# pierluigiferrari/ssd_keras

Hardware: AMD Instinct MI355X
Metric: images/sec SSD300 fwd+decode @batch32 (higher is better)
Workload: dtype f32 (decode, threshold, TF-style f32 NMS, top-k); bf16 conv backbone; 1 GPU; SSD300 VGG-16 inference (mode='inference': forward + DecodeDetections), 21 classes, batch 32 per GPU, conf 0.01 / NMS 0.45 / top-200, random-init weights, synthetic 300x300x3 uint8-range images; per_gpu_batch=32, global_batch=32, conv_dtype=bf16, parallelism=replicas x1, launch=hip_graph (forward + DecodeDetections captured once, replayed per step), decode_stream=same stream; DecodeDetections reads the head outputs directly (no y_pred in HBM)

## Files before the change

include/ssdhip.h:

```cpp
#ifndef SSDHIP_H
#define SSDHIP_H

#include <stddef.h>

#ifdef __cplusplus
extern "C" {
#endif

#define SSDHIP_ABI_VERSION 1

enum {
    SSDHIP_OK = 0,
    SSDHIP_E_BADARG = -1,
    SSDHIP_E_WORKSPACE = -2,
    SSDHIP_E_LAUNCH = -3
};

enum { SSDHIP_F32 = 0, SSDHIP_F64 = 1 };
enum { SSDHIP_CENTROIDS = 0, SSDHIP_CORNERS = 1, SSDHIP_MINMAX = 2 };
enum { SSDHIP_BORDER_HALF = 0, SSDHIP_BORDER_INCLUDE = 1, SSDHIP_BORDER_EXCLUDE = 2 };
enum {
    SSDHIP_SEM_NUMPY = 0,
    SSDHIP_SEM_KERAS = 1,
    SSDHIP_SEM_DEBUG = 2
};

int ssdhip_abi_version(void);
const char* ssdhip_strerror(int rc);

size_t ssdhip_decode_workspace_bytes(int B, int N, int C, int top_k, int nms_cap, int class_agnostic, int in_dtype);
int ssdhip_decode_detections(const void* y_pred, int in_dtype, int B, int N, int C,
                             double conf_thresh, double iou_thresh, int top_k, int nms_cap,
                             int class_agnostic, int semantics,
                             int coords, int normalize_coords, double img_height, double img_width,
                             int border_pixels,
                             void* out, int out_dtype, int out_rows, int* out_count, int* out_anchor_idx,
                             void* ws, size_t ws_bytes, void* stream);
int ssdhip_decode_stages(int stages, const void* y_pred, int in_dtype, int B, int N, int C,
                         double conf_thresh, double iou_thresh, int top_k, int nms_cap,
                         int class_agnostic, int semantics,
                         int coords, int normalize_coords, double img_height, double img_width,
                         int border_pixels,
                         void* out, int out_dtype, int out_rows, int* out_count, int* out_anchor_idx,
                         void* ws, size_t ws_bytes, void* stream);

size_t ssdhip_encode_workspace_bytes(int B, int N, int C, int G_total);
int ssdhip_encode(const double* anchors, const double* variances, const double* gt, const int* gt_offsets,
                  int G_total, int max_gt_per_image, int B, int N, int C, double img_height, double img_width,
                  int matching_type, double pos_iou_threshold, double neg_iou_limit,
                  int coords, int normalize_coords, int border_pixels, int background_id,
                  float* y_encoded_f32, double* y_encoded_f64, int* match_gt,
                  void* ws, size_t ws_bytes, void* stream);

// ... 488 lines not shown
```

ssd_keras_amd/_native.py:

```python
from __future__ import annotations

import ctypes
import os
import threading

import numpy as np

_LIB_PATH = os.environ.get("SSDHIP_LIB") or os.path.join(os.path.dirname(os.path.abspath(__file__)), "libssdhip.so")
_lib = None
_lock = threading.Lock()

F32, F64 = 0, 1
COORDS = {"centroids": 0, "corners": 1, "minmax": 2}
BORDER = {"half": 0, "include": 1, "exclude": 2}
SEM_NUMPY, SEM_KERAS, SEM_DEBUG = 0, 1, 2
ABI_VERSION = 1


class SsdHipError(RuntimeError):
    pass


def lib_path():
    return _LIB_PATH
# ... 33 lines not shown
                ("photo_prob", ctypes.c_double * 4), ("photo_lower", ctypes.c_double * 4), ("photo_upper", ctypes.c_double * 4),
                ("patch_prob", ctypes.c_double),
                ("min_scale", ctypes.c_double), ("max_scale", ctypes.c_double),
                ("min_aspect_ratio", ctypes.c_double), ("max_aspect_ratio", ctypes.c_double),
                ("n_trials", ctypes.c_int), ("clip_boxes", ctypes.c_int), ("criterion", ctypes.c_int), ("n_boxes_min", ctypes.c_int),
                ("validator_lower", ctypes.c_double), ("validator_upper", ctypes.c_double),
                ("filter_lower", ctypes.c_double), ("filter_upper", ctypes.c_double),
                ("flip_prob", ctypes.c_double),
                ("out_height", ctypes.c_int), ("out_width", ctypes.c_int), ("interpolation", ctypes.c_int),
                ("resize_min_area", ctypes.c_double)]


class _SatAugParams(ctypes.Structure):
    _fields_ = [("var", _VarAugParams), ("vflip_prob", ctypes.c_double), ("rotate_prob", ctypes.c_double)]


_I, _LL, _SZ, _D, _F, _P = ctypes.c_int, ctypes.c_longlong, ctypes.c_size_t, ctypes.c_double, ctypes.c_float, ctypes.c_void_p
_INTP, _PARAMS, _PHOTO = ctypes.POINTER(ctypes.c_int), ctypes.POINTER(_AugParams), ctypes.POINTER(_AugPhoto)
_LLP = ctypes.POINTER(ctypes.c_longlong)
SIGNATURES = {
    "ssdhip_abi_version": (_I, []),
    "ssdhip_strerror": (ctypes.c_char_p, [_I]),
    "ssdhip_decode_workspace_bytes": (_SZ, [_I] * 7),
    "ssdhip_decode_detections": (_I, [_P] + [_I] * 4 + [_D, _D] + [_I] * 6 + [_D, _D, _I, _P, _I, _I] + [_P] * 3 + [_SZ, _P]),
    "ssdhip_decode_stages": (_I, [_I, _P] + [_I] * 4 + [_D, _D] + [_I] * 6 + [_D, _D, _I, _P, _I, _I] + [_P] * 3 + [_SZ, _P]),
    "ssdhip_encode_workspace_bytes": (_SZ, [_I] * 4),
    "ssdhip_encode": (_I, [_P] * 4 + [_I] * 5 + [_D, _D, _I, _D, _D] + [_I] * 4 + [_P] * 4 + [_SZ, _P]),
    "ssdhip_loss_workspace_bytes": (_SZ, [_I] * 3),
    "ssdhip_loss_forward": (_I, [_P, _P] + [_I] * 5 + [_F] + [_P] * 4 + [_SZ, _P]),
    "ssdhip_loss_backward": (_I, [_P] * 5 + [_I] * 3 + [_F, _P, _P]),
    "ssdhip_convert_coordinates": (_I, [_P, _I, _P, _LL] + [_I] * 4 + [_P]),
    "ssdhip_iou_result_dtype": (_I, [_I] * 3),
    "ssdhip_box_overlap": (_I, [_I, _P, _I, _I, _P] + [_I] * 5 + [_P, _P]),
    "ssdhip_match_bipartite_greedy": (_I, [_P, _I, _I, _P, _P]),
    "ssdhip_match_multi_workspace_bytes": (_SZ, [_I, _I]),
    "ssdhip_match_multi": (_I, [_P, _I, _I, _D] + [_P] * 4 + [_SZ, _P]),
    "ssdhip_greedy_nms_workspace_bytes": (_SZ, [_I]),
    "ssdhip_greedy_nms": (_I, [_P] + [_I] * 4 + [_P, _I, _D, _I, _I] + [_P] * 3 + [_SZ, _P]),
    "ssdhip_box_filter": (_I, [_P] * 3 + [_I] * 6 + [_D] * 3 + [_I, _P, _P]),
    "ssdhip_match_predictions_workspace_bytes": (_SZ, [_I, _I]),
    "ssdhip_match_predictions": (_I, [_P, _P, _I] + [_P] * 3 + [_I, _I, _D, _I] + [_P] * 6 + [_SZ, _P]),
    "ssdhip_match_predictions_multi": (_I, [_P] * 3 + [_I] + [_P] * 3 + [_I, _I, _P, _I, _D, _I] + [_P] * 6 + [_SZ, _P]),
    "ssdhip_coco_match_workspace_bytes": (_SZ, [_I] * 4),
    "ssdhip_coco_match": (_I, [_P] * 3 + [_I] + [_P] * 4 + [_I, _I, _P, _I, _P, _I, _I] + [_P] * 8 + [_SZ, _P]),
    "ssdhip_coco_accumulate_workspace_bytes": (_SZ, [_I, _I]),
    "ssdhip_coco_accumulate": (_I, [_P] * 4 + [_I, _P, _P] + [_I] * 4 + [_P, _I, _I, _P, _I] + [_P] * 4 + [_SZ, _P]),
# ... 192 lines not shown
    check(rc, name)
    return True


def launch(name, device, *args):
    _launch(name, device, args)


def _launch_or_none(name, device, *args):
    return _launch(name, device, args, declines=True)


class _Workspaces:

    def __init__(self):
        self._bufs = {}

    def get(self, device, purpose, nbytes, zeroed=False):
        torch = _torch()
        key = (str(device), purpose, int(torch.cuda.current_stream(device).cuda_stream))
        buf = self._bufs.get(key)
        if buf is None or buf.numel() < nbytes:
            buf = (torch.zeros if zeroed else torch.empty)(int(nbytes), dtype=torch.uint8, device=device)
            self._bufs[key] = buf
        return buf


workspaces = _Workspaces()


def decode(y_pred, conf_thresh, iou_thresh, top_k, nms_cap, class_agnostic, semantics, coords, normalize_coords,
           img_height, img_width, border_pixels, out_dtype, out_rows, want_anchor_idx=False, workspace=None,
           stages=7, outputs=None):
    torch = _torch()
    lib = load()
    require_cuda(y_pred, "y_pred")
    if y_pred.dtype not in (torch.float32, torch.float64):
        raise SsdHipError("y_pred must be float32 or float64")
    in_dt = F32 if y_pred.dtype == torch.float32 else F64
    if in_dt == F64 and semantics == SEM_KERAS:
        raise SsdHipError("the DecodeDetections layers are float32 graphs: float64 predictions are not accepted there")
    B, N, L = y_pred.shape
    C = L - 12
    dev = y_pred.device
    k = int(top_k) if top_k else 0
    cap = int(nms_cap) if nms_cap else 0
    need = lib.ssdhip_decode_workspace_bytes(B, N, C, k, cap, int(bool(class_agnostic)), in_dt)
    if need == 0:
        raise SsdHipError("unsupported decode shape B=%d N=%d C=%d" % (B, N, C))
    ws = workspace if workspace is not None else workspaces.get(dev, "decode", need)
    if outputs is not None:
        out, count, aidx = outputs
    else:
        out = torch.empty((B, out_rows, 6), dtype=torch.float64 if out_dtype == F64 else torch.float32, device=dev)
        count = torch.empty((B,), dtype=torch.int32, device=dev)
        aidx = torch.empty((B, out_rows), dtype=torch.int32, device=dev) if want_anchor_idx else None
    launch("ssdhip_decode_stages", dev, int(stages), ctypes.c_void_p(y_pred.data_ptr()), in_dt, B, N, C, float(conf_thresh),
           float(iou_thresh), k, cap, int(bool(class_agnostic)), int(semantics), COORDS[coords], int(bool(normalize_coords)),
           float(img_height if img_height is not None else 1.0), float(img_width if img_width is not None else 1.0), BORDER[border_pixels],
           ctypes.c_void_p(out.data_ptr()), out_dtype, int(out_rows), ctypes.c_void_p(count.data_ptr()),
           ctypes.c_void_p(aidx.data_ptr()) if aidx is not None else None, ctypes.c_void_p(ws.data_ptr()), ws.numel())
    return out, count, aidx


def to_device(a, device=None, dtype=None):
    torch = _torch()
    if isinstance(a, np.ndarray):
        a = torch.from_numpy(np.ascontiguousarray(a))
    if device is None:
        device = a.device if a.is_cuda else torch.device("cuda", torch.cuda.current_device())
    if dtype is not None and a.dtype != dtype:
        a = a.to(dtype)
    return a.to(device, non_blocking=False).contiguous()




def _nhwc_bf16(t, name):
    torch = _torch()
    if not t.is_cuda or t.dtype != torch.bfloat16 or t.dim() != 4:
        raise SsdHipError("%s must be a 4-D bfloat16 CUDA tensor" % name)
    if not t.permute(0, 2, 3, 1).is_contiguous():
        t = t.contiguous(memory_format=torch.channels_last)
        if not t.permute(0, 2, 3, 1).is_contiguous():
# ... 223 lines not shown


def assemble_predictions(confs, locs, conf_biases, loc_biases, n_boxes, anchors_var, n_classes):
    torch = _torch()
    args, keep, B, N = _head_sources(confs, locs, conf_biases, loc_biases, n_boxes, anchors_var, n_classes)
    y = torch.empty((B, N, n_classes + 12), dtype=torch.float32, device=confs[0].device)
    f32 = confs[0].dtype == torch.float32
    launch("ssdhip_assemble_predictions_strided_" + ("f32" if f32 else "bf16"), y.device, *args, B, N, int(n_classes), _ptr(y))
    return y


def decode_from_heads(confs, locs, conf_biases, loc_biases, n_boxes, anchors_var, n_classes, conf_thresh, iou_thresh, top_k,
                      nms_cap, class_agnostic, semantics, coords, normalize_coords, img_height, img_width, border_pixels, out_dtype,
                      out_rows, want_anchor_idx=False):
    torch = _torch()
    lib = load()
    args, keep, B, N = _head_sources(confs, locs, conf_biases, loc_biases, n_boxes, anchors_var, n_classes)
    dev = confs[0].device
    k = int(top_k) if top_k else 0
    cap = int(nms_cap) if nms_cap else 0
    need = lib.ssdhip_decode_workspace_bytes(B, N, int(n_classes), k, cap, int(bool(class_agnostic)), F32)
    if need == 0:
        raise SsdHipError("unsupported decode shape B=%d N=%d C=%d" % (B, N, n_classes))
    ws = workspaces.get(dev, "decode", need)
    out = torch.empty((B, out_rows, 6), dtype=torch.float64 if out_dtype == F64 else torch.float32, device=dev)
    count = torch.empty((B,), dtype=torch.int32, device=dev)
    aidx = torch.empty((B, out_rows), dtype=torch.int32, device=dev) if want_anchor_idx else None
    launch("ssdhip_decode_from_heads_f32" if confs[0].dtype == torch.float32 else "ssdhip_decode_from_heads", dev, *args, B, N,
           int(n_classes), float(conf_thresh), float(iou_thresh), k, cap, int(bool(class_agnostic)), int(semantics), COORDS[coords],
           int(bool(normalize_coords)), float(img_height if img_height is not None else 1.0),
           float(img_width if img_width is not None else 1.0), BORDER[border_pixels], _ptr(out), out_dtype, int(out_rows), _ptr(count),
           _ptr(aidx), _ptr(ws), ws.numel())
    return out, count, aidx


def channel_sums_partial(gy):
    torch = _torch()
    lib = load()
    gy, (b, h, w, c) = _nhwc_bf16(gy, "gy")
    nb = lib.ssdhip_relu_bwd_bias_blocks(b * h * w, c)
    if nb == 0:
        return None
    partial = torch.empty((nb, c), dtype=torch.float32, device=gy.device)
    launch("ssdhip_channel_sums_nhwc_bf16", gy.device, _ptr(gy), _ptr(partial), b * h * w, c, nb)
    return partial


def relu_bwd_bias(gy, y, reduce=True):
    torch = _torch()
    lib = load()
    gy, (b, h, w, c) = _nhwc_bf16(gy, "gy")
    y, _ = _nhwc_bf16(y, "y")
    nb = lib.ssdhip_relu_bwd_bias_blocks(b * h * w, c)
    if nb == 0:
        return None
# ... 1994 lines not shown
```

ssd_keras_amd/csrc/ssdhip_decode.hip:

```cpp
#include <hip/hip_runtime.h>
#include <stdint.h>
#include <stdlib.h>

#include "ssdhip.h"
#include "ssdhip_math.h"
#include "ssdhip_tile.h"
#include "ssdhip_heads.h"
#include "ssdhip_decode64.h"

#ifdef SSDHIP_PROFILE
__device__ unsigned long long g_prof[64];
#define PROF_DECL long long _pt = clock64(); long long _pa[12] = {0, 0, 0, 0, 0, 0, 0, 0, 0, 0, 0, 0};
#define PROF_MARK(i) { const long long _t = clock64(); _pa[i] += _t - _pt; _pt = _t; }
#define PROF_FLUSH(base) if (threadIdx.x == 0) { for (int _i = 0; _i < 12; ++_i) if (_pa[_i]) atomicAdd(&g_prof[(base) + _i], (unsigned long long)_pa[_i]); }
extern "C" int ssdhip_profile_read(unsigned long long* host_out, int reset) {
    if (hipMemcpyFromSymbol(host_out, HIP_SYMBOL(g_prof), sizeof(g_prof)) != hipSuccess) return -1;
    if (reset) { unsigned long long z[64] = {0}; if (hipMemcpyToSymbol(HIP_SYMBOL(g_prof), z, sizeof(z)) != hipSuccess) return -1; }
    return 0;
}
#else
#define PROF_DECL
#define PROF_MARK(i)
#define PROF_FLUSH(base)
#endif

// ... 635 lines not shown
__device__ __forceinline__ void load_keys_cached(const u64* keys, int n, int tid, int first, u64 (&kc)[KP]) {
#if defined(__HIP_DEVICE_COMPILE__)
    int nn = n;
    asm volatile("" : "+s"(nn));
    const __amdgpu_buffer_rsrc_t rs = __builtin_amdgcn_make_buffer_rsrc(const_cast<u64*>(keys), 0, nn * 8, 0x00020000);
#pragma unroll
    for (int u = 0; u < KP; ++u) {
        const u32x2 v = __builtin_amdgcn_raw_buffer_load_b64(rs, tid * 8, (first + u) * T * 8, 0);
        const u64 key = ((u64)v.y << 32) | v.x;
        kc[u] = key ? key : ~0ull;
    }
#endif
}

__device__ __forceinline__ int uni32(int v) { return __builtin_amdgcn_readfirstlane(v); }
__device__ __forceinline__ u64 uni64(u64 v) {
    return ((u64)(u32)__builtin_amdgcn_readfirstlane((int)(u32)(v >> 32)) << 32) | (u64)(u32)__builtin_amdgcn_readfirstlane((int)(u32)v);
}

#ifndef SSDHIP_NMS_WAVES512
#define SSDHIP_NMS_WAVES512 6
#endif
template <int POL, int T, bool FULL>
__global__ __launch_bounds__(T, (T >= 512 ? SSDHIP_NMS_WAVES512 : 3)) void nms_kernel(DecodeParams p, const float4* __restrict__ boxes,
                                               const u64* __restrict__ cand, const int* __restrict__ cand_count,
                                               const int* __restrict__ work_order,
                                               u64* __restrict__ kept, int* __restrict__ kept_count, int redo_only) {
    constexpr int W = T / 64;
    constexpr int KC = KC_KEYS / T;
    constexpr int KP = 9;
    static_assert(KC % KP == 0, "KC must be a multiple of the trip size");
    constexpr int UA = T >= 512 ? (POL == POL_NUMPY64 ? 2 : 4) : 4, UB = T >= 512 ? 2 : 4;
    constexpr bool PREFETCH = T < 512;
    const int total_work = p.B * p.G;
    const int per_xcd = (total_work + 7) >> 3;
    int work = (blockIdx.x & 7) * per_xcd + (blockIdx.x >> 3);
    if ((int)(blockIdx.x >> 3) >= per_xcd || work >= total_work) return;
    if (work_order) work = work_order[work];
    if (redo_only && kept_count[work] != -1) return;
    const int b = work / p.G;

    __shared__ __attribute__((aligned(16))) u64 keybuf[MAX_CHUNK + 8];
    __shared__ __attribute__((aligned(16))) u64 keybuf2[MAX_CHUNK + 8];
    __shared__ int fill2;
    constexpr size_t SCRATCH = sizeof(FBox) * MAX_CHUNK > NMS_NBINS * sizeof(u32) ? sizeof(FBox) * MAX_CHUNK : NMS_NBINS * sizeof(u32);
    __shared__ __attribute__((aligned(16))) unsigned char scratch[SCRATCH];
    __shared__ __attribute__((aligned(16))) float4 cf4[POL == POL_NUMPY64 ? MAX_CHUNK : 1];
    __shared__ FBox kb[KEPT_LDS + 8 * W + 8];
    __shared__ __attribute__((aligned(16))) float4 kf4[POL == POL_NUMPY64 ? KEPT_LDS : 1];
    __shared__ u64 maskrow[64];
    __shared__ u64 supp_a[W];
    __shared__ int red[264];
    __shared__ int fill;
    u32* hist = reinterpret_cast<u32*>(scratch);
    FBox* cb = reinterpret_cast<FBox*>(scratch);
    u64* sorted = keybuf;

    const int tid = threadIdx.x, lane = tid & 63, wave = tid >> 6;
    const int n = cand_count[work];
    const u64* keys = cand + (size_t)work * p.N;
    u64* kept_out = kept + (size_t)work * p.cap_store;
    const float4* img_boxes = boxes + (size_t)b * p.N;
// ... 101 lines not shown
                    else if (m2 > 0 && bin >= bin_cut2) keybuf2[atomicAdd(&fill2, 1)] = key;
                }
            }
        } else {
            for (int i0 = tid; i0 < n; i0 += 8 * T) {
                u64 k8[8];
#pragma unroll
                for (int u = 0; u < 8; ++u) { const int i = i0 + u * T; k8[u] = i < n ? keys[i] : ~0ull; }
#pragma unroll
                for (int u = 0; u < 8; ++u) {
                    const u64 key = k8[u];
                    if (!(key < upper)) continue;
                    const int bin = bin_of<NMS_BIN_SHIFT, NMS_NBINS>((u32)(key >> IDX_BITS), p.thr_key);
                    const bool take = by_bin ? (bin >= bin_cut) : (key >= cutoff);
                    if (take) keybuf[atomicAdd(&fill, 1)] = key;
                    else if (m2 > 0 && bin >= bin_cut2) keybuf2[atomicAdd(&fill2, 1)] = key;
                }
            }
        }
        pending2 = m2;
        __syncthreads();
        PROF_MARK(1)
        }
        {
            constexpr int PER = MAX_CHUNK / T;
            u64 v[PER];
#pragma unroll
            for (int r = 0; r < PER; ++r) v[r] = keybuf[tid * PER + r];
            block_bitonic_desc_regs<T, PER>(v, reinterpret_cast<u64*>(scratch));
#pragma unroll
            for (int r = 0; r < PER; ++r) keybuf[tid * PER + r] = v[r];
            __syncthreads();
        }
        PROF_MARK(2)
        upper = uni64(sorted[m - 1]);
        has_upper = true;
        consumed += m;
        for (int i = tid; i < m; i += T) {
            const u32 idx = IDX_MASK - (u32)(sorted[i] & IDX_MASK);
            const float4 f4 = img_boxes[idx];
            cb[i] = make_fbox<POL>(f4, idx, k);
            if (POL == POL_NUMPY64) cf4[i] = f4;
        }
        __syncthreads();
        PROF_MARK(3)

        for (int base = 0; base < m && K < cap_eff && !finished; base += 64) {
            const int nb = min(64, m - base);
            const bool valid = lane < nb;
            const FBox me = cb[base + (valid ? lane : 0)];
            float4 me4 = make_float4(0.f, 0.f, 0.f, 0.f);
            if (POL == POL_NUMPY64) me4 = cf4[base + (valid ? lane : 0)];
            bool supp = false;
            if (!k.no_nms) {
                const int Kl = min(K, KEPT_LDS);
// ... 132 lines not shown
            const bool keep_me = (alive >> lane) & 1ull;
            if (wave == 0 && keep_me) {
                const int pos = K + __popcll(alive & lanemask_lt());
                kept_out[pos] = sorted[base + dl];
                if (pos < KEPT_LDS) {
                    kb[pos] = cb[base + dl];
                    if (POL == POL_NUMPY64) kf4[pos] = cf4[base + dl];
                }
            }
            K += cnt;
            if (POL != POL_TF32 && !k.no_nms) {
                const float a_me = keep_me ? cb[base + dl].area : 0.f;
                if (__ballot(keep_me && a_me != a_me)) finished = true;
            }
            __syncthreads();
            PROF_MARK(6)
        }
    }
    PROF_FLUSH(0)
#ifdef SSDHIP_PROFILE
    if (tid == 0) { atomicAdd(&g_prof[12], 1ull); atomicAdd(&g_prof[13], (unsigned long long)consumed); atomicAdd(&g_prof[14], (unsigned long long)K); }
#endif
    if (tid == 0) kept_count[work] = K;
}

template <typename OutT>
__device__ __forceinline__ void write_row(OutT* out, int* out_idx, int row, int cls, u64 key, const float4* img_boxes,
                                          const DecodeParams& p) {
    const u32 idx = IDX_MASK - (u32)(key & IDX_MASK);
    const float s = key_float((u32)(key >> IDX_BITS));
    const float4 bx = img_boxes[idx];
    OutT* r = out + (size_t)row * 6;
    r[0] = (OutT)cls;
    r[1] = (OutT)s;
    if (p.iou_f32) {
        r[2] = (OutT)(bx.x * (float)p.img_w);
        r[3] = (OutT)(bx.y * (float)p.img_h);
        r[4] = (OutT)(bx.z * (float)p.img_w);
        r[5] = (OutT)(bx.w * (float)p.img_h);
    } else {
        r[2] = (OutT)((double)bx.x * p.img_w);
        r[3] = (OutT)((double)bx.y * p.img_h);
        r[4] = (OutT)((double)bx.z * p.img_w);
        r[5] = (OutT)((double)bx.w * p.img_h);
    }
    if (out_idx) out_idx[row] = (int)idx;
}

__device__ __forceinline__ int find_group(const int* offs, int G, int e) {
    int lo = 0, hi = G;
    while (hi - lo > 1) {
        const int mid = (lo + hi) >> 1;
        if (offs[mid] <= e) lo = mid; else hi = mid;
    }
    return lo;
}

constexpr int TOPK_THREADS = 1024;

template <typename OutT>
__global__ __launch_bounds__(TOPK_THREADS) void topk_kernel(DecodeParams p, const float4* __restrict__ boxes,
                                                            const u64* __restrict__ kept, const int* __restrict__ kept_count,
                                                            const unsigned short* __restrict__ cls_map,
                                                            OutT* __restrict__ out, int* __restrict__ out_count,
                                                            int* __restrict__ out_idx, int sort_cap) {
    constexpr int T5 = TOPK_THREADS;
    extern __shared__ __attribute__((aligned(16))) unsigned char smem_raw[];
    u64* buf = reinterpret_cast<u64*>(smem_raw);
    u32* hist = reinterpret_cast<u32*>(smem_raw);
    int* offs = reinterpret_cast<int*>(smem_raw + (size_t)sort_cap * sizeof(u64));
    __shared__ int red[260];
    __shared__ int fill;
    __shared__ int wave_tot[T5 / 64];
    __shared__ u32 tie_lo, tie_hi;

    const int b = blockIdx.x, tid = threadIdx.x, lane = tid & 63, wave = tid >> 6;
    const int G = p.G;
    const float4* img_boxes = boxes + (size_t)b * p.N;
    const u64* img_kept = kept + (size_t)b * G * p.cap_store;
    OutT* img_out = out + (size_t)b * p.out_rows * 6;
    int* img_idx = out_idx ? out_idx + (size_t)b * p.out_rows : nullptr;
    const unsigned short* img_cls = p.class_agnostic ? cls_map + (size_t)b * p.N : nullptr;

    {
        int run = 0;
        for (int g0 = 0; g0 < G; g0 += T5) {
            const int g = g0 + tid;
            const int c = g < G ? kept_count[b * G + g] : 0;
            int inc = c;
            for (int off = 1; off < 64; off <<= 1) { const int o = __shfl_up(inc, off); if (lane >= off) inc += o; }
            if (lane == 63) wave_tot[wave] = inc;
            __syncthreads();
            int before = run;
            for (int w = 0; w < wave; ++w) before += wave_tot[w];
            if (g < G) offs[g] = before + inc - c;
            for (int w = 0; w < T5 / 64; ++w) run += wave_tot[w];
            __syncthreads();
        }
        if (tid == 0) offs[G] = run;
    }
    PROF_DECL
    __syncthreads();
    PROF_MARK(0)
    const int T = offs[G];
    int rows = p.top_k > 0 ? min(T, p.top_k) : T;
    rows = min(rows, p.out_rows);

    auto comp_of = [&](int g, int r) -> u64 {
        const u64 key = img_kept[(size_t)g * p.cap_store + r];
        const u32 pos = (u32)g * (u32)p.cap_store + (u32)r;
        return ((key >> IDX_BITS) << 32) | (u64)(0xffffffffu - pos);
// ... 177 lines not shown
                u64 cm2 = 0;
                bool sel = false;
                if (e < T) { cm2 = comp_at(e); sel = cm2 >= cutoff; }
                const u64 m = __ballot(sel);
                if (lane == 0) wave_tot[wave] = __popcll(m);
                __syncthreads();
                int off = base;
                for (int w = 0; w < wave; ++w) off += wave_tot[w];
                if (sel) emit(off + __popcll(m & lanemask_lt()), cm2);
                for (int w = 0; w < T5 / 64; ++w) base += wave_tot[w];
                __syncthreads();
            }
        }
    }
    PROF_MARK(4)
    for (int i = rows * 6 + tid; i < p.out_rows * 6; i += T5) img_out[i] = (OutT)0;
    if (img_idx) for (int i = rows + tid; i < p.out_rows; i += T5) img_idx[i] = -1;
    if (tid == 0) out_count[b] = rows;
    PROF_MARK(5)
    PROF_FLUSH(32)
}

struct DecodeWs {
    size_t boxes, cand_count, kept_count, cls, cand, kept, total;
};

static inline size_t align_up(size_t v, size_t a) { return (v + a - 1) / a * a; }

static int cap_store_for(int N, int top_k, int nms_cap) {
    int cap = N;
    if (nms_cap > 0) cap = nms_cap < cap ? nms_cap : cap;
    if (top_k > 0) cap = top_k < cap ? top_k : cap;
    return cap < 1 ? 1 : cap;
}

static DecodeWs decode_ws_layout(int B, int N, int C, int top_k, int nms_cap, int class_agnostic) {
    const size_t G = class_agnostic ? 1 : (size_t)(C - 1);
    const size_t cap = (size_t)cap_store_for(N, top_k, nms_cap);
    DecodeWs w;
    size_t o = 0;
    w.boxes = o;      o = align_up(o + (size_t)B * N * sizeof(float4), 256);
    w.cand_count = o; o = align_up(o + (size_t)B * G * sizeof(int), 256);
    w.kept_count = o; o = align_up(o + (size_t)B * G * sizeof(int), 256);
    w.cls = o;        o = align_up(o + (class_agnostic ? (size_t)B * N * sizeof(unsigned short) : 0), 256);
    w.cand = o;       o = align_up(o + (size_t)B * G * N * sizeof(u64), 256);
    w.kept = o;       o = align_up(o + (size_t)B * G * cap * sizeof(u64), 256);
    w.total = o;
    return w;
}

}

using namespace ssdhip;

extern "C" size_t ssdhip_decode_workspace_bytes(int B, int N, int C, int top_k, int nms_cap, int class_agnostic, int in_dtype) {
    if (B <= 0 || N <= 0 || C < 2 || (in_dtype != SSDHIP_F32 && in_dtype != SSDHIP_F64)) return 0;
    if (in_dtype == SSDHIP_F64) return decode64_workspace_bytes(B, N, C, top_k, nms_cap, class_agnostic);
    return decode_ws_layout(B, N, C, top_k, nms_cap, class_agnostic).total;
}

struct HeadSource {
    const HeadParams* hp;
    const float* anchors_var;
    int tiles;
};

static int decode_run(const HeadSource* heads, int stages, const void* y_pred, int in_dtype, int B, int N, int C,
                      double conf_thresh, double iou_thresh, int top_k, int nms_cap,
                      int class_agnostic, int semantics,
                      int coords, int normalize_coords, double img_height, double img_width,
                      int border_pixels,
                      void* out, int out_dtype, int out_rows, int* out_count, int* out_anchor_idx,
                      void* ws, size_t ws_bytes, void* stream_) {
    hipStream_t stream = static_cast<hipStream_t>(stream_);
    if ((!y_pred && !heads) || !out || !out_count || B <= 0 || N <= 0 || C < 2 || out_rows <= 0) return SSDHIP_E_BADARG;
    if (in_dtype != SSDHIP_F32 && in_dtype != SSDHIP_F64) return SSDHIP_E_BADARG;
    if (out_dtype != SSDHIP_F32 && out_dtype != SSDHIP_F64) return SSDHIP_E_BADARG;
    if (N > (1 << IDX_BITS) || C > 1025) return SSDHIP_E_BADARG;
    if (coords < 0 || coords > 2 || border_pixels < 0 || border_pixels > 2) return SSDHIP_E_BADARG;
    if (semantics < 0 || semantics > 2) return SSDHIP_E_BADARG;
    if (in_dtype == SSDHIP_F64) {
// ... 27 lines not shown
        cv.f = te;
        const unsigned key = (cv.u & 0x80000000u) ? ~cv.u : (cv.u | 0x80000000u);
        p.thr_key = key;
    }
    p.iou_thresh = iou_thresh;
    p.img_w = normalize_coords ? img_width : 1.0;
    p.img_h = normalize_coords ? img_height : 1.0;
    p.fast_ok = (iou_thresh > 0.0 && iou_thresh < 1e300) ? 1 : 0;
    if (semantics == SSDHIP_SEM_KERAS) p.fast_ok = ((float)iou_thresh >= 1e-30f && (float)iou_thresh < 1e30f) ? 1 : 0;
    p.px_f32 = (semantics == SSDHIP_SEM_KERAS) ? 1 : 0;
    p.no_nms = (iou_thresh == (double)INFINITY) ? 1 : 0;
    p.filter_kE = (iou_thresh > 0.0 && iou_thresh <= 16.0) ? (float)((16.0 + 40.0 * iou_thresh) * 0x1p-24 * 1.001) : INFINITY;
    if (p.px_f32 && ((double)(float)p.img_w != p.img_w || (double)(float)p.img_h != p.img_h)) return SSDHIP_E_BADARG;
    p.top_k = top_k; p.cap = nms_cap; p.cap_store = cap_store_for(N, top_k, nms_cap);
    p.out_rows = out_rows; p.sorted = sorted;

    unsigned char* base = static_cast<unsigned char*>(ws);
    float4* boxes = reinterpret_cast<float4*>(base + lay.boxes);
    int* cand_count = reinterpret_cast<int*>(base + lay.cand_count);
    int* kept_count = reinterpret_cast<int*>(base + lay.kept_count);
    unsigned short* cls_map = reinterpret_cast<unsigned short*>(base + lay.cls);
    u64* cand = reinterpret_cast<u64*>(base + lay.cand);
    u64* kept = reinterpret_cast<u64*>(base + lay.kept);

    if (stages & 1) {
    if (zero_async(cand_count, (size_t)B * p.G * sizeof(int), stream) != hipSuccess) return SSDHIP_E_LAUNCH;

    int TA = 256;
    while (TA > 64 && (size_t)TA * p.L * sizeof(float) > 24 * 1024) TA >>= 1;
    size_t k3_lds = align_up(((size_t)TA * p.L + 4) * sizeof(float), 16) + (size_t)(TA / 64) * p.G * sizeof(int);
    k3_lds = k3_lds > align_up((size_t)TA * p.L * sizeof(float), 1024) ? k3_lds : align_up((size_t)TA * p.L * sizeof(float), 1024);
    { const char* e = getenv("SSDHIP_SCAN_DMA"); p.no_dma = (e && e[0] == '0') ? 1 : 0; }
    if (k3_lds > 160 * 1024) return SSDHIP_E_BADARG;
    if (heads) {
        const int HT = heads->hp->TA;
        const size_t lds = (head_tile_lds(HT, C) + 15) / 16 * 16 + (size_t)((HT + 63) / 64) * p.G * sizeof(int);
        if (lds > 160 * 1024) return SSDHIP_E_BADARG;
        const char* rows_env = getenv("SSDHIP_SCAN_ROWS");
        const bool rows_lds = rows_env && rows_env[0] == 'l' && rows_env[1] == 'd' && rows_env[2] == 's' && !rows_env[3];
        if (!rows_lds && C == 21 && HT == 256 && heads->hp->C == C && head_rows_all_dma(*heads->hp, B, HT, heads->anchors_var)) {
            const size_t rlds = (head_stage_bytes(HT, C) + 15) / 16 * 16 + (size_t)(HT / 64) * p.G * sizeof(int);
            hipLaunchKernelGGL(scan_heads_rows_kernel<21>, dim3(heads->tiles, B), dim3(HT), rlds, stream, *heads->hp, heads->anchors_var,
                               p, boxes, cand, cand_count, cls_map);
        } else
        hipLaunchKernelGGL(scan_heads_kernel, dim3(heads->tiles, B), dim3(HT < 64 ? 64 : HT), lds, stream, *heads->hp,
                           heads->anchors_var, p, boxes, cand, cand_count, cls_map);
    } else if (p.L > 64 && !p.class_agnostic) {
        dim3 g3((N + SW_WAVES * 64 - 1) / (SW_WAVES * 64), B);
        hipLaunchKernelGGL(scan_wide_kernel, g3, dim3(SW_WAVES * 64), 0, stream, static_cast<const float*>(y_pred), p, boxes, cand, cand_count);
    } else {
        dim3 g3((N + TA - 1) / TA, B);
        hipLaunchKernelGGL(scan_kernel, g3, dim3(TA), k3_lds, stream, static_cast<const float*>(y_pred), p, boxes, cand,
                           cand_count, cls_map);
    }
    if (hipGetLastError() != hipSuccess) return SSDHIP_E_LAUNCH;
    }

    if (stages & 2) {
    const int work = B * p.G;
    const int g4 = ((work + 7) / 8) * 8;
    const int* order = nullptr;
    static const int nms_env = []() { const char* e = getenv("SSDHIP_NMS_T"); return e ? atoi(e) : 0; }();
    const int nms_t = nms_env ? nms_env : (semantics == SSDHIP_SEM_KERAS ? 512 : 256);
#define SSDHIP_LAUNCH_NMS(POL)                                                                                                            \
    do {                                                                                                                                  \
        if (nms_t >= 512) {                                                                                                               \
            hipLaunchKernelGGL((nms_kernel<POL, 512, false>), dim3(g4), dim3(512), 0, stream, p, boxes, cand, cand_count, order, kept, kept_count, 0); \
            hipLaunchKernelGGL((nms_kernel<POL, 512, true>), dim3(g4), dim3(512), 0, stream, p, boxes, cand, cand_count, order, kept, kept_count, 1); \
        } else {                                                                                                                          \
            hipLaunchKernelGGL((nms_kernel<POL, 256, true>), dim3(g4), dim3(256), 0, stream, p, boxes, cand, cand_count, order, kept, kept_count, 0); \
        }                                                                                                                                 \
    } while (0)
    if (semantics == SSDHIP_SEM_KERAS) SSDHIP_LAUNCH_NMS(POL_TF32);
    else if (p.iou_f32) SSDHIP_LAUNCH_NMS(POL_NUMPY32);
    else SSDHIP_LAUNCH_NMS(POL_NUMPY64);
#undef SSDHIP_LAUNCH_NMS
    if (hipGetLastError() != hipSuccess) return SSDHIP_E_LAUNCH;
    }

    if (stages & 4) {
    size_t sort_cap = 4096;
    while (sort_cap < (size_t)p.G * (size_t)p.cap_store && sort_cap < 16384) sort_cap <<= 1;
    const size_t k5_lds = sort_cap * sizeof(u64) + align_up((size_t)(p.G + 1) * sizeof(int), 16);
    const void* fn = out_dtype == SSDHIP_F32 ? reinterpret_cast<const void*>(topk_kernel<float>) : reinterpret_cast<const void*>(topk_kernel<double>);
    if (k5_lds > 48 * 1024 && hipFuncSetAttribute(fn, hipFuncAttributeMaxDynamicSharedMemorySize, (int)k5_lds) != hipSuccess) return SSDHIP_E_LAUNCH;
    if (out_dtype == SSDHIP_F32)
        hipLaunchKernelGGL(topk_kernel<float>, dim3(B), dim3(TOPK_THREADS), k5_lds, stream, p, boxes, kept, kept_count, cls_map,
                           static_cast<float*>(out), out_count, out_anchor_idx, (int)sort_cap);
    else
        hipLaunchKernelGGL(topk_kernel<double>, dim3(B), dim3(TOPK_THREADS), k5_lds, stream, p, boxes, kept, kept_count, cls_map,
                           static_cast<double*>(out), out_count, out_anchor_idx, (int)sort_cap);
    if (hipGetLastError() != hipSuccess) return SSDHIP_E_LAUNCH;
    }
    return SSDHIP_OK;
}

extern "C" int ssdhip_decode_detections(const void* y_pred, int in_dtype, int B, int N, int C,
                                        double conf_thresh, double iou_thresh, int top_k, int nms_cap,
                                        int class_agnostic, int semantics,
                                        int coords, int normalize_coords, double img_height, double img_width,
                                        int border_pixels,
                                        void* out, int out_dtype, int out_rows, int* out_count, int* out_anchor_idx,
                                        void* ws, size_t ws_bytes, void* stream) {
    return decode_run(nullptr, 7, y_pred, in_dtype, B, N, C, conf_thresh, iou_thresh, top_k, nms_cap, class_agnostic, semantics, coords,
                      normalize_coords, img_height, img_width, border_pixels, out, out_dtype, out_rows, out_count,
                      out_anchor_idx, ws, ws_bytes, stream);
}

extern "C" int ssdhip_decode_stages(int stages, const void* y_pred, int in_dtype, int B, int N, int C,
                                    double conf_thresh, double iou_thresh, int top_k, int nms_cap,
                                    int class_agnostic, int semantics,
                                    int coords, int normalize_coords, double img_height, double img_width,
                                    int border_pixels,
                                    void* out, int out_dtype, int out_rows, int* out_count, int* out_anchor_idx,
// ... 57 lines not shown
```

Baseline: 17170 images/sec.

## Fold NMS redo pass into top-k kernel and self-reset live counters

Drops the per-call memset of candidate counts. A separate 'live' counter region in the workspace is now zeroed by the top-k kernel after it reads the counts, with a Python context manager tracking workspace state and issuing a one-time reset when needed. In the whole-pipeline Keras path, the second NMS launch (redo of overflowed groups) is removed and its work runs inside the top-k kernel through a shared nms_work device function using 1024 threads. Together this removes two launches from the captured graph. The cost is extra state-tracking complexity, a serial per-group redo inside a single block per image, and higher LDS and register pressure in topk_kernel.

```diff
diff --git a/include/ssdhip.h b/include/ssdhip.h
--- a/include/ssdhip.h
+++ b/include/ssdhip.h
@@ -29,6 +29,8 @@
 const char* ssdhip_strerror(int rc);
 
 size_t ssdhip_decode_workspace_bytes(int B, int N, int C, int top_k, int nms_cap, int class_agnostic, int in_dtype);
+int ssdhip_decode_workspace_reset(void* ws, size_t ws_bytes, int B, int N, int C, int top_k, int nms_cap, int class_agnostic,
+                                  void* stream);
 int ssdhip_decode_detections(const void* y_pred, int in_dtype, int B, int N, int C,
                              double conf_thresh, double iou_thresh, int top_k, int nms_cap,
                              int class_agnostic, int semantics,
diff --git a/ssd_keras_amd/_native.py b/ssd_keras_amd/_native.py
--- a/ssd_keras_amd/_native.py
+++ b/ssd_keras_amd/_native.py
@@ -79,6 +79,7 @@
     "ssdhip_abi_version": (_I, []),
     "ssdhip_strerror": (ctypes.c_char_p, [_I]),
     "ssdhip_decode_workspace_bytes": (_SZ, [_I] * 7),
+    "ssdhip_decode_workspace_reset": (_I, [_P, _SZ] + [_I] * 6 + [_P]),
     "ssdhip_decode_detections": (_I, [_P] + [_I] * 4 + [_D, _D] + [_I] * 6 + [_D, _D, _I, _P, _I, _I] + [_P] * 3 + [_SZ, _P]),
     "ssdhip_decode_stages": (_I, [_I, _P] + [_I] * 4 + [_D, _D] + [_I] * 6 + [_D, _D, _I, _P, _I, _I] + [_P] * 3 + [_SZ, _P]),
     "ssdhip_encode_workspace_bytes": (_SZ, [_I] * 4),
@@ -317,11 +318,56 @@
         buf = self._bufs.get(key)
         if buf is None or buf.numel() < nbytes:
             buf = (torch.zeros if zeroed else torch.empty)(int(nbytes), dtype=torch.uint8, device=device)
+            if zeroed and purpose == "decode":
+                setattr(buf, _DecodeWorkspace.ATTR, _DecodeWorkspace.ZEROED)
             self._bufs[key] = buf
         return buf
 
 
 workspaces = _Workspaces()
+
+
+class _DecodeWorkspace:
+    ATTR, PINNED = "_ssdhip_decode_state", "_ssdhip_decode_pinned"
+    ZEROED = "zeroed"
+
+    def __init__(self, device, nbytes, layout, whole=True, f32=True, workspace=None):
+        torch = _torch()
+        self.device, self.layout, self.whole, self.f32 = device, tuple(int(v) for v in layout), whole, f32
+        capturing = torch.cuda.is_current_stream_capturing()
+        if workspace is not None:
+            self.ws = workspace
+        else:
+            self.ws = workspaces.get(device, "decode", nbytes, zeroed=not capturing)
+            pinned = getattr(self.ws, self.PINNED, None)
+            if capturing and whole and f32 and pinned is not None and pinned != self.layout:
+                self.ws = workspaces.get(device, ("decode",) + self.layout, nbytes)
+        if capturing and whole and f32:
+            setattr(self.ws, self.PINNED, self.layout)
+
+    def _reset(self, layout):
+        launch("ssdhip_decode_workspace_reset", self.device, _ptr(self.ws), self.ws.numel(), *layout)
+
+    def __enter__(self):
+        state = getattr(self.ws, self.ATTR, None)
+        self.after = self.layout
+        if not self.f32:
+            self.after = None
+        elif not self.whole:
+            self.after = state if state == self.layout else None
+        elif state != self.ZEROED and state != self.layout:
+            self._reset(self.layout)
+        setattr(self.ws, self.ATTR, None)
+        return self.ws
+
+    def __exit__(self, exc_type, exc, tb):
+        if exc_type is None:
+            pinned = getattr(self.ws, self.PINNED, None)
+            if pinned is not None and self.after != pinned:
+                self._reset(pinned)
+                self.after = pinned
+            setattr(self.ws, self.ATTR, self.after)
+        return False
 
 
 def decode(y_pred, conf_thresh, iou_thresh, top_k, nms_cap, class_agnostic, semantics, coords, normalize_coords,
@@ -343,18 +389,19 @@
     need = lib.ssdhip_decode_workspace_bytes(B, N, C, k, cap, int(bool(class_agnostic)), in_dt)
     if need == 0:
         raise SsdHipError("unsupported decode shape B=%d N=%d C=%d" % (B, N, C))
-    ws = workspace if workspace is not None else workspaces.get(dev, "decode", need)
     if outputs is not None:
         out, count, aidx = outputs
     else:
         out = torch.empty((B, out_rows, 6), dtype=torch.float64 if out_dtype == F64 else torch.float32, device=dev)
         count = torch.empty((B,), dtype=torch.int32, device=dev)
         aidx = torch.empty((B, out_rows), dtype=torch.int32, device=dev) if want_anchor_idx else None
-    launch("ssdhip_decode_stages", dev, int(stages), ctypes.c_void_p(y_pred.data_ptr()), in_dt, B, N, C, float(conf_thresh),
-           float(iou_thresh), k, cap, int(bool(class_agnostic)), int(semantics), COORDS[coords], int(bool(normalize_coords)),
-           float(img_height if img_height is not None else 1.0), float(img_width if img_width is not None else 1.0), BORDER[border_pixels],
-           ctypes.c_void_p(out.data_ptr()), out_dtype, int(out_rows), ctypes.c_void_p(count.data_ptr()),
-           ctypes.c_void_p(aidx.data_ptr()) if aidx is not None else None, ctypes.c_void_p(ws.data_ptr()), ws.numel())
+    with _DecodeWorkspace(dev, need, (B, N, C, k, cap, bool(class_agnostic)), whole=int(stages) == 7, f32=in_dt == F32,
+                          workspace=workspace) as ws:
+        launch("ssdhip_decode_stages", dev, int(stages), ctypes.c_void_p(y_pred.data_ptr()), in_dt, B, N, C, float(conf_thresh),
+               float(iou_thresh), k, cap, int(bool(class_agnostic)), int(semantics), COORDS[coords], int(bool(normalize_coords)),
+               float(img_height if img_height is not None else 1.0), float(img_width if img_width is not None else 1.0),
+               BORDER[border_pixels], ctypes.c_void_p(out.data_ptr()), out_dtype, int(out_rows), ctypes.c_void_p(count.data_ptr()),
+               ctypes.c_void_p(aidx.data_ptr()) if aidx is not None else None, ctypes.c_void_p(ws.data_ptr()), ws.numel())
     return out, count, aidx
 
 
@@ -624,15 +671,15 @@
     need = lib.ssdhip_decode_workspace_bytes(B, N, int(n_classes), k, cap, int(bool(class_agnostic)), F32)
     if need == 0:
         raise SsdHipError("unsupported decode shape B=%d N=%d C=%d" % (B, N, n_classes))
-    ws = workspaces.get(dev, "decode", need)
     out = torch.empty((B, out_rows, 6), dtype=torch.float64 if out_dtype == F64 else torch.float32, device=dev)
     count = torch.empty((B,), dtype=torch.int32, device=dev)
     aidx = torch.empty((B, out_rows), dtype=torch.int32, device=dev) if want_anchor_idx else None
-    launch("ssdhip_decode_from_heads_f32" if confs[0].dtype == torch.float32 else "ssdhip_decode_from_heads", dev, *args, B, N,
-           int(n_classes), float(conf_thresh), float(iou_thresh), k, cap, int(bool(class_agnostic)), int(semantics), COORDS[coords],
-           int(bool(normalize_coords)), float(img_height if img_height is not None else 1.0),
-           float(img_width if img_width is not None else 1.0), BORDER[border_pixels], _ptr(out), out_dtype, int(out_rows), _ptr(count),
-           _ptr(aidx), _ptr(ws), ws.numel())
+    with _DecodeWorkspace(dev, need, (B, N, int(n_classes), k, cap, bool(class_agnostic))) as ws:
+        launch("ssdhip_decode_from_heads_f32" if confs[0].dtype == torch.float32 else "ssdhip_decode_from_heads", dev, *args, B, N,
+               int(n_classes), float(conf_thresh), float(iou_thresh), k, cap, int(bool(class_agnostic)), int(semantics), COORDS[coords],
+               int(bool(normalize_coords)), float(img_height if img_height is not None else 1.0),
+               float(img_width if img_width is not None else 1.0), BORDER[border_pixels], _ptr(out), out_dtype, int(out_rows),
+               _ptr(count), _ptr(aidx), _ptr(ws), ws.numel())
     return out, count, aidx
 
 
diff --git a/ssd_keras_amd/csrc/ssdhip_decode.hip b/ssd_keras_amd/csrc/ssdhip_decode.hip
--- a/ssd_keras_amd/csrc/ssdhip_decode.hip
+++ b/ssd_keras_amd/csrc/ssdhip_decode.hip
@@ -1,6 +1,8 @@
 #include <hip/hip_runtime.h>
 #include <stdint.h>
 #include <stdlib.h>
+#include <string.h>
+#include <type_traits>
 
 #include "ssdhip.h"
 #include "ssdhip_math.h"
@@ -682,22 +684,15 @@
 #define SSDHIP_NMS_WAVES512 6
 #endif
 template <int POL, int T, bool FULL>
-__global__ __launch_bounds__(T, (T >= 512 ? SSDHIP_NMS_WAVES512 : 3)) void nms_kernel(DecodeParams p, const float4* __restrict__ boxes,
-                                               const u64* __restrict__ cand, const int* __restrict__ cand_count,
-                                               const int* __restrict__ work_order,
-                                               u64* __restrict__ kept, int* __restrict__ kept_count, int redo_only) {
+__device__ __forceinline__ void nms_work(const DecodeParams& p, const float4* __restrict__ boxes, const u64* __restrict__ cand,
+                                         const int* __restrict__ cand_count, u64* __restrict__ kept, int* __restrict__ kept_count,
+                                         const int work) {
     constexpr int W = T / 64;
     constexpr int KC = KC_KEYS / T;
     constexpr int KP = 9;
     static_assert(KC % KP == 0, "KC must be a multiple of the trip size");
     constexpr int UA = T >= 512 ? (POL == POL_NUMPY64 ? 2 : 4) : 4, UB = T >= 512 ? 2 : 4;
     constexpr bool PREFETCH = T < 512;
-    const int total_work = p.B * p.G;
-    const int per_xcd = (total_work + 7) >> 3;
-    int work = (blockIdx.x & 7) * per_xcd + (blockIdx.x >> 3);
-    if ((int)(blockIdx.x >> 3) >= per_xcd || work >= total_work) return;
-    if (work_order) work = work_order[work];
-    if (redo_only && kept_count[work] != -1) return;
     const int b = work / p.G;
 
     __shared__ __attribute__((aligned(16))) u64 keybuf[MAX_CHUNK + 8];
@@ -845,7 +840,7 @@
         __syncthreads();
         PROF_MARK(1)
         }
-        {
+        if constexpr (T <= MAX_CHUNK) {
             constexpr int PER = MAX_CHUNK / T;
             u64 v[PER];
 #pragma unroll
@@ -854,6 +849,8 @@
 #pragma unroll
             for (int r = 0; r < PER; ++r) keybuf[tid * PER + r] = v[r];
             __syncthreads();
+        } else {
+            block_bitonic_desc<T>(keybuf, MAX_CHUNK);
         }
         PROF_MARK(2)
         upper = uni64(sorted[m - 1]);
@@ -1032,6 +1029,20 @@
     if (tid == 0) { atomicAdd(&g_prof[12], 1ull); atomicAdd(&g_prof[13], (unsigned long long)consumed); atomicAdd(&g_prof[14], (unsigned long long)K); }
 #endif
     if (tid == 0) kept_count[work] = K;
+}
+
+template <int POL, int T, bool FULL>
+__global__ __launch_bounds__(T, (T >= 512 ? SSDHIP_NMS_WAVES512 : 3)) void nms_kernel(DecodeParams p, const float4* __restrict__ boxes,
+                                               const u64* __restrict__ cand, const int* __restrict__ cand_count,
+                                               const int* __restrict__ work_order,
+                                               u64* __restrict__ kept, int* __restrict__ kept_count, int redo_only) {
+    const int total_work = p.B * p.G;
+    const int per_xcd = (total_work + 7) >> 3;
+    int work = (blockIdx.x & 7) * per_xcd + (blockIdx.x >> 3);
+    if ((int)(blockIdx.x >> 3) >= per_xcd || work >= total_work) return;
+    if (work_order) work = work_order[work];
+    if (redo_only && kept_count[work] != -1) return;
+    nms_work<POL, T, FULL>(p, boxes, cand, cand_count, kept, kept_count, work);
 }
 
 template <typename OutT>
@@ -1067,14 +1078,31 @@
 }
 
 constexpr int TOPK_THREADS = 1024;
-
-template <typename OutT>
+constexpr int TOPK_NO_REDO = -1;
+
+template <typename OutT, int REDO>
 __global__ __launch_bounds__(TOPK_THREADS) void topk_kernel(DecodeParams p, const float4* __restrict__ boxes,
-                                                            const u64* __restrict__ kept, const int* __restrict__ kept_count,
+                                                            std::conditional_t<REDO >= 0, u64*, const u64* __restrict__> kept,
+                                                            const int* __restrict__ kept_count,
                                                             const unsigned short* __restrict__ cls_map,
                                                             OutT* __restrict__ out, int* __restrict__ out_count,
-                                                            int* __restrict__ out_idx, int sort_cap) {
+                                                            int* __restrict__ out_idx, int sort_cap,
+                                                            int* __restrict__ live_cand, int* __restrict__ live_kept,
+                                                            int* __restrict__ left_cand, int* __restrict__ left_kept,
+                                                            const u64* __restrict__ cand) {
     constexpr int T5 = TOPK_THREADS;
+    if constexpr (REDO >= 0) {
+        const int b = blockIdx.x, G = p.G;
+        int flagged = 0;
+        for (int g = threadIdx.x; g < G; g += T5) flagged |= live_kept[b * G + g] == -1;
+        if (__syncthreads_or(flagged)) {
+            for (int g = 0; g < G; ++g) {
+                if (live_kept[b * G + g] != -1) continue;
+                nms_work<REDO, T5, true>(p, boxes, cand, live_cand, kept, live_kept, b * G + g);
+                __syncthreads();
+            }
+        }
+    }
     extern __shared__ __attribute__((aligned(16))) unsigned char smem_raw[];
     u64* buf = reinterpret_cast<u64*>(smem_raw);
     u32* hist = reinterpret_cast<u32*>(smem_raw);
@@ -1096,7 +1124,13 @@
         int run = 0;
         for (int g0 = 0; g0 < G; g0 += T5) {
             const int g = g0 + tid;
-            const int c = g < G ? kept_count[b * G + g] : 0;
+            const int c = g < G ? (live_cand ? live_kept[b * G + g] : kept_count[b * G + g]) : 0;
+            if (live_cand && g < G) {
+                left_kept[b * G + g] = c;
+                left_cand[b * G + g] = live_cand[b * G + g];
+                live_kept[b * G + g] = 0;
+                live_cand[b * G + g] = 0;
+            }
             int inc = c;
             for (int off = 1; off < 64; off <<= 1) { const int o = __shfl_up(inc, off); if (lane >= off) inc += o; }
             if (lane == 63) wave_tot[wave] = inc;
@@ -1320,7 +1354,7 @@
 }
 
 struct DecodeWs {
-    size_t boxes, cand_count, kept_count, cls, cand, kept, total;
+    size_t boxes, cand_count, kept_count, cls, cand, kept, live, live_bytes, total;
 };
 
 static inline size_t align_up(size_t v, size_t a) { return (v + a - 1) / a * a; }
@@ -1343,6 +1377,8 @@
     w.cls = o;        o = align_up(o + (class_agnostic ? (size_t)B * N * sizeof(unsigned short) : 0), 256);
     w.cand = o;       o = align_up(o + (size_t)B * G * N * sizeof(u64), 256);
     w.kept = o;       o = align_up(o + (size_t)B * G * cap * sizeof(u64), 256);
+    w.live = o;       w.live_bytes = 2 * (size_t)B * G * sizeof(int);
+    o = align_up(o + w.live_bytes, 256);
     w.total = o;
     return w;
 }
@@ -1355,6 +1391,26 @@
     if (B <= 0 || N <= 0 || C < 2 || (in_dtype != SSDHIP_F32 && in_dtype != SSDHIP_F64)) return 0;
     if (in_dtype == SSDHIP_F64) return decode64_workspace_bytes(B, N, C, top_k, nms_cap, class_agnostic);
     return decode_ws_layout(B, N, C, top_k, nms_cap, class_agnostic).total;
+}
+
+static bool decode_launches_legacy() {
+    const char* e = getenv("SSDHIP_DECODE_LAUNCHES");
+    return e && !strcmp(e, "legacy");
+}
+
+extern "C" int ssdhip_decode_workspace_reset(void* ws, size_t ws_bytes, int B, int N, int C, int top_k, int nms_cap, int class_agnostic,
+                                             void* stream) {
+    if (B <= 0 || N <= 0 || C < 2) return SSDHIP_E_BADARG;
+    const DecodeWs lay = decode_ws_layout(B, N, C, top_k, nms_cap, class_agnostic);
+    if (!ws || ws_bytes < lay.total) return SSDHIP_E_WORKSPACE;
+    if (zero_async(static_cast<unsigned char*>(ws) + lay.live, lay.live_bytes, static_cast<hipStream_t>(stream)) != hipSuccess)
+        return SSDHIP_E_LAUNCH;
+    return SSDHIP_OK;
+}
+
+static size_t topk_static_lds(const void* fn) {
+    hipFuncAttributes a;
+    return hipFuncGetAttributes(&a, fn) == hipSuccess ? a.sharedSizeBytes : (size_t)1 << 30;
 }
 
 struct HeadSource {
@@ -1428,9 +1484,16 @@
     unsigned short* cls_map = reinterpret_cast<unsigned short*>(base + lay.cls);
     u64* cand = reinterpret_cast<u64*>(base + lay.cand);
     u64* kept = reinterpret_cast<u64*>(base + lay.kept);
+    int* const left_cand = cand_count;
+    int* const left_kept = kept_count;
+    const bool whole = stages == 7 && !decode_launches_legacy();
+    if (whole) {
+        cand_count = reinterpret_cast<int*>(base + lay.live);
+        kept_count = cand_count + (size_t)B * p.G;
+    }
 
     if (stages & 1) {
-    if (zero_async(cand_count, (size_t)B * p.G * sizeof(int), stream) != hipSuccess) return SSDHIP_E_LAUNCH;
+    if (!whole && zero_async(cand_count, (size_t)B * p.G * sizeof(int), stream) != hipSuccess) return SSDHIP_E_LAUNCH;
 
     int TA = 256;
     while (TA > 64 && (size_t)TA * p.L * sizeof(float) > 24 * 1024) TA >>= 1;
@@ -1462,16 +1525,28 @@
     if (hipGetLastError() != hipSuccess) return SSDHIP_E_LAUNCH;
     }
 
+    size_t sort_cap = 4096;
+    while (sort_cap < (size_t)p.G * (size_t)p.cap_store && sort_cap < 16384) sort_cap <<= 1;
+    const size_t k5_lds = sort_cap * sizeof(u64) + align_up((size_t)(p.G + 1) * sizeof(int), 16);
+    bool k5_redo = false;
+    if (whole && semantics == SSDHIP_SEM_KERAS) {
+        static const size_t redo_static[2] = {topk_static_lds(reinterpret_cast<const void*>(topk_kernel<float, POL_TF32>)),
+                                              topk_static_lds(reinterpret_cast<const void*>(topk_kernel<double, POL_TF32>))};
+        k5_redo = redo_static[out_dtype == SSDHIP_F32 ? 0 : 1] + k5_lds <= 160 * 1024;
+    }
+
     if (stages & 2) {
     const int work = B * p.G;
     const int g4 = ((work + 7) / 8) * 8;
     const int* order = nullptr;
     static const int nms_env = []() { const char* e = getenv("SSDHIP_NMS_T"); return e ? atoi(e) : 0; }();
     const int nms_t = nms_env ? nms_env : (semantics == SSDHIP_SEM_KERAS ? 512 : 256);
+    if (nms_t < 512) k5_redo = false;
 #define SSDHIP_LAUNCH_NMS(POL)                                                                                                            \
     do {                                                                                                                                  \
         if (nms_t >= 512) {                                                                                                               \
             hipLaunchKernelGGL((nms_kernel<POL, 512, false>), dim3(g4), dim3(512), 0, stream, p, boxes, cand, cand_count, order, kept, kept_count, 0); \
+            if (!k5_redo)                                                                                                                 \
             hipLaunchKernelGGL((nms_kernel<POL, 512, true>), dim3(g4), dim3(512), 0, stream, p, boxes, cand, cand_count, order, kept, kept_count, 1); \
         } else {                                                                                                                          \
             hipLaunchKernelGGL((nms_kernel<POL, 256, true>), dim3(g4), dim3(256), 0, stream, p, boxes, cand, cand_count, order, kept, kept_count, 0); \
@@ -1485,17 +1560,20 @@
     }
 
     if (stages & 4) {
-    size_t sort_cap = 4096;
-    while (sort_cap < (size_t)p.G * (size_t)p.cap_store && sort_cap < 16384) sort_cap <<= 1;
-    const size_t k5_lds = sort_cap * sizeof(u64) + align_up((size_t)(p.G + 1) * sizeof(int), 16);
-    const void* fn = out_dtype == SSDHIP_F32 ? reinterpret_cast<const void*>(topk_kernel<float>) : reinterpret_cast<const void*>(topk_kernel<double>);
-    if (k5_lds > 48 * 1024 && hipFuncSetAttribute(fn, hipFuncAttributeMaxDynamicSharedMemorySize, (int)k5_lds) != hipSuccess) return SSDHIP_E_LAUNCH;
-    if (out_dtype == SSDHIP_F32)
-        hipLaunchKernelGGL(topk_kernel<float>, dim3(B), dim3(TOPK_THREADS), k5_lds, stream, p, boxes, kept, kept_count, cls_map,
-                           static_cast<float*>(out), out_count, out_anchor_idx, (int)sort_cap);
-    else
-        hipLaunchKernelGGL(topk_kernel<double>, dim3(B), dim3(TOPK_THREADS), k5_lds, stream, p, boxes, kept, kept_count, cls_map,
-                           static_cast<double*>(out), out_count, out_anchor_idx, (int)sort_cap);
+    int* const live_cand = whole ? cand_count : nullptr;
+    int* const live_kept = whole ? kept_count : nullptr;
+#define SSDHIP_LAUNCH_TOPK(OUT_T, REDO)                                                                                                   \
+    do {                                                                                                                                  \
+        const void* fn = reinterpret_cast<const void*>(topk_kernel<OUT_T, REDO>);                                                         \
+        if (k5_lds > 48 * 1024 && hipFuncSetAttribute(fn, hipFuncAttributeMaxDynamicSharedMemorySize, (int)k5_lds) != hipSuccess)         \
+            return SSDHIP_E_LAUNCH;                                                                                                       \
+        hipLaunchKernelGGL((topk_kernel<OUT_T, REDO>), dim3(B), dim3(TOPK_THREADS), k5_lds, stream, p, boxes, kept, kept_count, cls_map,  \
+                           static_cast<OUT_T*>(out), out_count, out_anchor_idx, (int)sort_cap, live_cand, live_kept, left_cand,           \
+                           left_kept, cand);                                                                                              \
+    } while (0)
+    if (out_dtype == SSDHIP_F32) { if (k5_redo) SSDHIP_LAUNCH_TOPK(float, POL_TF32); else SSDHIP_LAUNCH_TOPK(float, TOPK_NO_REDO); }
+    else { if (k5_redo) SSDHIP_LAUNCH_TOPK(double, POL_TF32); else SSDHIP_LAUNCH_TOPK(double, TOPK_NO_REDO); }
+#undef SSDHIP_LAUNCH_TOPK
     if (hipGetLastError() != hipSuccess) return SSDHIP_E_LAUNCH;
     }
     return SSDHIP_OK;
```

Result: no change. 17250 images/sec, median of 6 (+0.4%).
